# opendilab/DI-engine

Hardware: NVIDIA H100
Metric: learner transitions/sec (GAE+ppo_error fwd+bwd, T=128 x B=4096 per GPU) (higher is better)
Workload: dtype f32

## Files before the change

__graft_entry__.py:

```python
import os
import subprocess
import sys

ROOT = os.path.dirname(os.path.abspath(__file__))
if ROOT not in sys.path:
    sys.path.insert(0, ROOT)

CSRC = os.path.join(ROOT, 'di-engine_b200', 'csrc')
LIBDIR = os.path.join(ROOT, 'di-engine_b200', 'lib')
SOURCES = ['api.cu', 'gae.cu', 'ppo.cu', 'td.cu', 'pg.cu', 'fused.cu', 'colws.cu', 'vtws.cu', 'policy.cu', 'heads.cu',
           'quantile.cu', 'retrace.cu', 'acer.cu', 'vocab.cu', 'scatter.cu', 'lstm.cu']
ARCH = ['-gencode', 'arch=compute_90a,code=sm_90a']
NVCC_FLAGS = ARCH + [
    '-O3', '-lineinfo', '-std=c++17', '-Xcompiler', '-fPIC',
    '-Xcompiler', '-fvisibility=hidden', '--expt-extended-lambda'
]


def _stale(out, deps):
    if not os.path.isfile(out):
        return True
    t = os.path.getmtime(out)
    return any(os.path.getmtime(d) > t for d in deps)


def build(force=False):
    nvcc = os.environ.get('NVCC', 'nvcc')
    os.makedirs(LIBDIR, exist_ok=True)
    hdrs = [os.path.join(CSRC, h) for h in ('common.cuh', 'gae_tile.cuh', 'ppo_math.cuh', 'fused_args.cuh', 'policy_stats.cuh')]
    hdrs.append(os.path.join(ROOT, 'include', 'b200rl.h'))
    objs = []
    procs = []
    for src in SOURCES:
        s = os.path.join(CSRC, src)
        o = os.path.join(CSRC, src[:-3] + '.o')
        objs.append(o)
        if force or _stale(o, [s] + hdrs):
            procs.append((src, subprocess.Popen([nvcc] + NVCC_FLAGS + ['-c', s, '-o', o])))
    for src, p in procs:
        if p.wait() != 0:
            raise RuntimeError('nvcc failed on ' + src)
    out = os.path.join(LIBDIR, 'libb200rl.so')
    if force or procs or _stale(out, objs):
        subprocess.check_call([nvcc] + ARCH + ['-shared', '-o', out] + objs +
                              ['-lcudart'])
    build_c_example(force=force or bool(procs))
    from oracle import make_ref, ref_coma, ref_lm, ref_scatter
    make_ref.build()
    ref_lm.build()
    ref_coma.build()
    ref_scatter.build()
    import di_engine_b200
    lib = di_engine_b200._lib.load()
    assert lib.b200rl_built_for_sm() == 90
    return out


def build_c_example(force=False):
    src = os.path.join(ROOT, 'examples', 'c_abi_gae.c')
    exe = os.path.join(ROOT, 'examples', 'bin', 'c_abi_gae')
    lib = os.path.join(LIBDIR, 'libb200rl.so')
    if not force and not _stale(exe, [src, lib, os.path.join(ROOT, 'include', 'b200rl.h')]):
        return exe
    os.makedirs(os.path.dirname(exe), exist_ok=True)
    cuda = os.environ.get('CUDA_HOME', '/usr/local/cuda')
    subprocess.check_call([
        os.environ.get('CC', 'gcc'), '-std=c11', '-O2', '-ffp-contract=off', '-I', os.path.join(ROOT, 'include'), '-I',
        os.path.join(cuda, 'include'), src, '-L', LIBDIR, '-lb200rl', '-L', os.path.join(cuda, 'lib64'), '-lcudart',
        '-Wl,-rpath,$ORIGIN/../../di-engine_b200/lib', '-Wl,-rpath,' + os.path.join(cuda, 'lib64'), '-o', exe
    ])
    return exe


def smoke():
    import numpy as np
    import torch
    import di_engine_b200 as b2
    from oracle import rl_oracle
    from tests import cases
    assert torch.cuda.is_available(), 'smoke() needs a GPU'
    T, B, N = 128, 64, 6
    op, tg, pg = cases.gae_case(1, T, B, p_done=0.02)
# ... 32 lines not shown
```

di-engine_b200/csrc/policy.cu:

```cuda
#include <math.h>

#include "../../include/b200rl.h"
#include "policy_stats.cuh"

namespace b200rl {

constexpr int GS_NT = 1024;
constexpr int GS_MAX_T = 24576;

template <int VN>
__global__ void __launch_bounds__(GS_NT) gae_seq_kernel(const float* __restrict__ value, float* __restrict__ next_value,
                                                       const float* __restrict__ reward, const float* __restrict__ done,
                                                       const float* __restrict__ traj, float* __restrict__ adv, int T,
                                                       float gamma, float gl, int mask_inplace, RetArgs ra) {
    pdl_prologue();
    extern __shared__ float s_seq[];
    float* s_d = s_seq;
    float* s_f = s_seq + T;
    __shared__ int s_nseg;
    __shared__ int s_cnt[GS_NT / 32];
    const int tid = threadIdx.x;
    const float vs = ra.vscale;
    float mu = 0.f, sigma = 1.f;
    if constexpr (VN == VN_POPART) {
        mu = *ra.mu;
        sigma = *ra.sigma;
    }
    for (int t = tid; t < T; t += GS_NT) {
        const float v = vn_decode<VN>(value[t], vs);
        float nv = vn_decode<VN>(next_value[t], vs);
        float r = reward[t];
        if constexpr (VN == VN_POPART) r = __fdiv_rn(fsub(r, mu), sigma);
        const float d = done ? done[t] : 0.f;
        const float tf = traj ? traj[t] : d;
        if (done) {
            nv = fmul(nv, fsub(1.f, d));
            if (VN == VN_PPO && mask_inplace && d != 0.f) next_value[t] = nv;
        }
        s_d[t] = fsub(fadd(r, fmul(gamma, nv)), v);
        s_f[t] = fmul(gl, fsub(1.f, tf));
    }
    __syncthreads();
    const int strip = (T + GS_NT - 1) / GS_NT;
    const int t0 = tid * strip, t1 = min(T, t0 + strip);
    int mine = 0;
    for (int t = t0; t < t1; ++t) mine += (s_f[t] == 0.f || t == T - 1) ? 1 : 0;
    int incl = mine;
    const int lane = tid & 31, wid = tid >> 5;
#pragma unroll
    for (int o = 1; o < 32; o <<= 1) {
        const int n = __shfl_up_sync(0xffffffffu, incl, o);
        if (lane >= o) incl += n;
    }
    if (lane == 31) s_cnt[wid] = incl;
    __syncthreads();
// ... 92 lines not shown
    pdl_prologue();
    const float vs = ra.vscale;
    double acc[4] = {0.0, 0.0, 0.0, 0.0}, pv[2];
    const long long stride = (long long)gridDim.x * 256;
    long long i = (long long)blockIdx.x * 256 + threadIdx.x;
    if (VEC) {
        const long long n4 = n >> 2;
        const float4* v4 = reinterpret_cast<const float4*>(value);
        const float4* a4 = reinterpret_cast<const float4*>(adv);
        float4 v = make_float4(0.f, 0.f, 0.f, 0.f), a = v;
        if (i < n4) {
            v = v4[i];
            a = a4[i];
        }
        ret_pivots<VN>(vs, ret_value<VN>(ld_after_wait(value), vs), ld_after_wait(adv), pv);
        for (; i < n4; i += stride) {
            float4 ru, vo, ro;
            ret_one<VN>(vs, v.x, a.x, ru.x, vo.x, ro.x, acc, pv);
            ret_one<VN>(vs, v.y, a.y, ru.y, vo.y, ro.y, acc, pv);
            ret_one<VN>(vs, v.z, a.z, ru.z, vo.z, ro.z, acc, pv);
            ret_one<VN>(vs, v.w, a.w, ru.w, vo.w, ro.w, acc, pv);
            if (ra.ret_unnorm) reinterpret_cast<float4*>(ra.ret_unnorm)[i] = ru;
            if (ra.value_out) reinterpret_cast<float4*>(ra.value_out)[i] = vo;
            if (ra.ret_out) reinterpret_cast<float4*>(ra.ret_out)[i] = ro;
            if (i + stride < n4) {
                v = v4[i + stride];
                a = a4[i + stride];
            }
        }
    } else {
        float v = 0.f, a = 0.f;
        if (i < n) {
            v = value[i];
            a = adv[i];
        }
        ret_pivots<VN>(vs, ret_value<VN>(ld_after_wait(value), vs), ld_after_wait(adv), pv);
        for (; i < n; i += stride) {
            float ru, vo, ro;
            ret_one<VN>(vs, v, a, ru, vo, ro, acc, pv);
            if (ra.ret_unnorm) ra.ret_unnorm[i] = ru;
            if (ra.value_out) ra.value_out[i] = vo;
            if (ra.ret_out) ra.ret_out[i] = ro;
            if (i + stride < n) {
                v = value[i + stride];
                a = adv[i + stride];
            }
        }
    }
    if (!ra.stats && !ra.adv_stats) return;
    double tot[4];
    if (stats_grid_join<4, 256>(acc, tot, ws_part, ws_join)) write_ret_stats<VN>(ra, tot, pv, (double)n);
}

__global__ void __launch_bounds__(256) adv_stats_kernel(const float* __restrict__ x, long long n, float* __restrict__ out,
                                                        double* __restrict__ ws_part, unsigned int* __restrict__ ws_join) {
    pdl_prologue();
    const double p = stats_pivot(ld_after_wait(x));
    double acc[2] = {0.0, 0.0};
    for (long long i = (long long)blockIdx.x * 256 + threadIdx.x; i < n; i += (long long)gridDim.x * 256)
        moments_add(acc[0], acc[1], x[i], p);
    double tot[2];
    if (stats_grid_join<2, 256>(acc, tot, ws_part, ws_join)) write_adv_stats(out, tot[0], tot[1], p, (double)n);
}

__global__ void __launch_bounds__(256) normalize_kernel(const float* __restrict__ x, const float* __restrict__ stats,
                                                        long long n, float* __restrict__ out) {
    pdl_prologue();
    const float m = ld_after_wait(stats), d = ld_after_wait(stats + 1);
    for (long long i = (long long)blockIdx.x * 256 + threadIdx.x; i < n; i += (long long)gridDim.x * 256)
        out[i] = __fdiv_rn(fsub(x[i], m), d);
}

__global__ void __launch_bounds__(256) impala_mask_kernel(const float* __restrict__ values, const float* __restrict__ rewards,
                                                          const float* __restrict__ done, long long T, long long B,
                                                          float* __restrict__ values_out, float* __restrict__ rewards_out,
                                                          float* __restrict__ weights_out) {
    pdl_prologue();
    const long long n = (T + 1) * B;
    for (long long i = (long long)blockIdx.x * 256 + threadIdx.x; i < n; i += (long long)gridDim.x * 256) {
        const long long t = i / B;
        const float m = t >= 1 ? fsub(1.f, done[i - B]) : 1.f;
        values_out[i] = t >= 1 ? fmul(values[i], m) : values[i];
        if (t < T) {
            if (weights_out) weights_out[i] = m;
            if (rewards_out) rewards_out[i] = fmul(rewards[i], m);
        }
    }
}

enum ValueMap : int { VM_SYMLOG = 0, VM_INV_SYMLOG = 1, VM_H_INV = 2, VM_POPART_REWARD = 3 };

template <int M>
__device__ __forceinline__ float value_map(float x, float mu, float sigma) {
    if constexpr (M == VM_SYMLOG) return vn_symlog(x);
    else if constexpr (M == VM_INV_SYMLOG) return vn_inv_symlog(x);
    else if constexpr (M == VM_H_INV) return vn_h_inv(x);
    else return __fdiv_rn(fsub(x, mu), sigma);
}

template <int M>
__global__ void __launch_bounds__(256) value_map_kernel(const float* __restrict__ x0, float* __restrict__ y0,
                                                        const float* __restrict__ x1, float* __restrict__ y1, long long n,
                                                        const float* __restrict__ mu, const float* __restrict__ sigma) {
    pdl_prologue();
    float m = 0.f, sg = 1.f;
    if constexpr (M == VM_POPART_REWARD) {
        m = *mu;
        sg = *sigma;
    }
    for (long long i = (long long)blockIdx.x * 256 + threadIdx.x; i < n; i += (long long)gridDim.x * 256) {
        y0[i] = value_map<M>(x0[i], m, sg);
        if (x1) y1[i] = value_map<M>(x1[i], m, sg);
    }
}

template <int M>
__global__ void __launch_bounds__(256) value_map_bwd_kernel(const float* __restrict__ x, const float* __restrict__ g,
                                                            float* __restrict__ dx, long long n) {
    pdl_prologue();
    for (long long i = (long long)blockIdx.x * 256 + threadIdx.x; i < n; i += (long long)gridDim.x * 256) {
        const float xi = x[i], s = vn_sign(xi), gs = fmul(g[i], s);
        const float d = M == VM_SYMLOG ? __fdiv_rn(gs, fadd(fabsf(xi), 1.f)) : fmul(gs, expf(fabsf(xi)));
        dx[i] = fadd(0.f, fmul(d, s));
    }
}

}

using namespace b200rl;

namespace b200rl {
int gae_scan(const float* value, float* next_value, const float* reward, const float* done, const float* traj_flag, float* adv,
             long long T, long long C, long long A, double gamma_d, double lambda_d, int mask_next_value_inplace,
             float vscale, void* stream);
}

static double* ws_stats_part(float* ws) { return reinterpret_cast<double*>(ws + WS_CTRL_WORDS); }
static unsigned int* ws_joins(float* ws) { return reinterpret_cast<unsigned int*>(ws + WS_FX_OFF_WORDS + 48); }
static_assert(WS_CTRL_WORDS % 2 == 0 && WS_CTRL_WORDS + NUM_SMS * 8 * 4 * 2 <= WS_PARTIAL_LIMIT_WORDS,
              "the statistics rows fit the workspace's partial region");

extern "C" int b200rl_adv_stats(const float* x, long long n, float* stats2, float* workspace, size_t workspace_bytes,
                                void* stream) {
    if (!x || !stats2 || !workspace || n < 1 || workspace_bytes < WS_MIN_BYTES) return B200RL_ERR_ARG;
    long long grid = div_up(n, 256 * 8);
    if (grid > NUM_SMS * 4) grid = NUM_SMS * 4;
    if (grid < 1) grid = 1;
    return launch_k(adv_stats_kernel, (int)grid, 256, 0, (cudaStream_t)stream, x, n, stats2, ws_stats_part(workspace),
                    ws_joins(workspace));
}

extern "C" int b200rl_normalize(const float* x, const float* stats2, long long n, float* out, void* stream) {
    if (!x || !stats2 || !out || n < 0) return B200RL_ERR_ARG;
    if (n == 0) return B200RL_OK;
    long long grid = div_up(n, 256 * 4);
    if (grid > NUM_SMS * 8) grid = NUM_SMS * 8;
    return launch_k(normalize_kernel, (int)grid, 256, 0, (cudaStream_t)stream, x, stats2, n, out);
}

extern "C" int b200rl_gae_returns(const float* value, float* next_value, const float* reward, const float* done,
                                  const float* traj_flag, long long T, long long C, long long A, double gamma,
                                  double lambda_, int mask_next_value_inplace, double value_scale, float* adv,
                                  float* unnormalized_return, float* value_out, float* return_out, float* stats3,
                                  float* adv_stats2, float* workspace, size_t workspace_bytes, void* stream) {
    if (T < 1 || C < 1 || A < 1 || !value || !next_value || !reward || !adv || !workspace ||
        workspace_bytes < WS_MIN_BYTES || value_scale < 0.0)
        return B200RL_ERR_ARG;
    RetArgs ra{};
    ra.vscale = (float)value_scale;
    ra.ret_unnorm = unnormalized_return; ra.value_out = value_out; ra.ret_out = return_out; ra.stats = stats3;
    ra.adv_stats = adv_stats2;
    cudaStream_t st = (cudaStream_t)stream;
    if (C == 1 && T <= GS_MAX_T) {
        const size_t smem = (size_t)2 * T * sizeof(float);
        if (int rc = smem_opt_in<gae_seq_kernel<VN_PPO>>(smem)) return rc;
        return launch_k(gae_seq_kernel<VN_PPO>, 1, GS_NT, smem, st, value, next_value, reward, done, traj_flag, adv, (int)T,
                        (float)gamma, (float)(gamma * lambda_), mask_next_value_inplace, ra);
    }
    const bool want_epi = unnormalized_return || value_out || return_out || stats3 || adv_stats2;
    int rc = gae_scan(value, next_value, reward, done, traj_flag, adv, T, C, A, gamma, lambda_, mask_next_value_inplace,
                      (float)value_scale, stream);
    if (rc != 0 || !want_epi) return rc;
    const long long n = T * C;
    const bool vec = (n % 4 == 0) && aligned16(value) && aligned16(adv) && (!unnormalized_return || aligned16(unnormalized_return)) &&
                     (!value_out || aligned16(value_out)) && (!return_out || aligned16(return_out));
    long long grid = div_up(n, 256 * (vec ? 8 : 4));
    if (grid > NUM_SMS * 8) grid = NUM_SMS * 8;
    if (vec)
        return launch_k(returns_kernel<VN_PPO, true>, (int)grid, 256, 0, st, value, (const float*)adv, n, ra,
                        ws_stats_part(workspace), ws_joins(workspace));
    return launch_k(returns_kernel<VN_PPO, false>, (int)grid, 256, 0, st, value, (const float*)adv, n, ra,
                    ws_stats_part(workspace), ws_joins(workspace));
}

static long long map_grid(long long n) {
    long long grid = div_up(n, 256 * 4);
    if (grid > NUM_SMS * 8) grid = NUM_SMS * 8;
    return grid < 1 ? 1 : grid;
}

template <int VN>
static int launch_gae_seq(const float* value, const float* next_value, const float* reward, const float* done,
                          const float* traj_flag, float* adv, long long T, double gamma, double lambda_, const RetArgs& ra,
                          cudaStream_t st) {
    const size_t smem = (size_t)2 * T * sizeof(float);
    if (int rc = smem_opt_in<gae_seq_kernel<VN>>(smem)) return rc;
    return launch_k(gae_seq_kernel<VN>, 1, GS_NT, smem, st, value, const_cast<float*>(next_value), reward, done, traj_flag,
                    adv, (int)T, (float)gamma, (float)(gamma * lambda_), 0, ra);
}

template <int VN>
static int launch_returns(const float* value, const float* adv, long long n, const RetArgs& ra, float* workspace,
                          cudaStream_t st) {
    const bool vec = (n % 4 == 0) && aligned16(value) && aligned16(adv) && (!ra.value_out || aligned16(ra.value_out)) &&
                     (!ra.ret_out || aligned16(ra.ret_out));
    long long grid = div_up(n, 256 * (vec ? 8 : 4));
    if (grid > NUM_SMS * 8) grid = NUM_SMS * 8;
    if (vec)
        return launch_k(returns_kernel<VN, true>, (int)grid, 256, 0, st, value, adv, n, ra, ws_stats_part(workspace),
                        ws_joins(workspace));
    return launch_k(returns_kernel<VN, false>, (int)grid, 256, 0, st, value, adv, n, ra, ws_stats_part(workspace),
                    ws_joins(workspace));
}

template <int VN>
static int launch_gae_returns_tc(const float* value, const float* next_value, const float* reward, const float* done,
                                 const float* traj_flag, float* adv, long long T, long long C, double gamma, double lambda_,
                                 const RetArgs& ra, float* scratch, float* workspace, cudaStream_t st) {
    const long long n = T * C;
    const float* v = value;
    const float* nv = next_value;
    const float* r = reward;
    int rc = 0;
    if constexpr (VN == VN_RESCALE || VN == VN_SYMLOG) {
        constexpr int M = VN == VN_RESCALE ? VM_H_INV : VM_INV_SYMLOG;
        rc = launch_k(value_map_kernel<M>, (int)map_grid(n), 256, 0, st, value, scratch, next_value, scratch + n, n,
                      (const float*)nullptr, (const float*)nullptr);
        v = scratch;
        nv = scratch + n;
    } else if constexpr (VN == VN_POPART) {
        rc = launch_k(value_map_kernel<VM_POPART_REWARD>, (int)map_grid(n), 256, 0, st, reward, scratch,
                      (const float*)nullptr, (float*)nullptr, n, ra.mu, ra.sigma);
        r = scratch;
    }
    if (rc) return rc;
// ... 81 lines not shown
```

di-engine_b200/csrc/ppo.cu:

```cuda
#include "../../include/b200rl.h"
#include "ppo_math.cuh"

namespace b200rl {

constexpr int PS_CW = 8;
constexpr int PS_R = PS_CW * 32;
constexpr int PS_THREADS = PS_R + 32;
constexpr int PS_MAX_STAGES = 8;
constexpr int PS_AHEAD = 2;
constexpr size_t PS_SMEM_LIMIT = 227 * 1024 - 1024;
constexpr int PS_TRACE_STAGES = 56;

template <int NC, int WHAT>
__global__ void __launch_bounds__(PS_THREADS, 1) ppo_tile_kernel(PpoArgs a, float* ws, int n_stages, int trace) {
    extern __shared__ __align__(128) unsigned char smem[];
    unsigned long long* tr = trace ? reinterpret_cast<unsigned long long*>(ws + 65536) + blockIdx.x * 64 : nullptr;
    if (tr && threadIdx.x == 0) tr[0] = gtimer();
    pdl_prologue();
    if (tr && threadIdx.x == 0) tr[1] = gtimer();
    constexpr bool GRADS = (WHAT != PPO_FWD);
    constexpr bool LOSSES = (WHAT != PPO_BWD);
    const int N = NC ? NC : a.N;
    const int tid = threadIdx.x;
    const int wid = tid >> 5, lane = tid & 31;
    const bool has_pre = a.logit_pre != nullptr, has_w = a.weight != nullptr;
    const PpoTileLayout L = ppo_layout(N, has_pre, has_w, PS_R);
    const int NS = n_stages;
    uint64_t* full = reinterpret_cast<uint64_t*>(smem + NS * L.stage_bytes);
    uint64_t* empty = full + PS_MAX_STAGES;

    float g[4] = {0.f, 0.f, 0.f, 0.f};
    if (GRADS && upstream<4>(a.rec, WHAT == PPO_BWD, ppo_owned(a), g)) return;
    const PpoUpstream up{g[0], g[1], g[2], g[3], 1.f / (float)a.S};

    const long long n_full = a.S / PS_R;
    const int tail_rows = (int)(a.S - n_full * PS_R);
    const long long n_tiles = n_full + (tail_rows ? 1 : 0);
    const long long t0 = n_tiles * blockIdx.x / gridDim.x, t1 = n_tiles * (blockIdx.x + 1) / gridDim.x;
    const int my_n = (int)(t1 - t0);

    if (tid == 0) {
        for (int s = 0; s < NS; ++s) {
            mbar_init(&full[s], 1);
            mbar_init(&empty[s], PS_CW);
        }
        mbar_fence_init();
    }
    __syncthreads();

    float acc[6] = {0.f, 0.f, 0.f, 0.f, 0.f, 0.f};
    if (wid == PS_CW) {
        if (lane == 0) {
            for (int i = 0; i < my_n; ++i) {
                const long long t = t0 + i;
                if (t >= n_full) break;
                const int sg = i % NS;
                if (i >= NS) mbar_wait(&empty[sg], (uint32_t)(((i / NS) - 1) & 1));
                if (NS > PS_AHEAD && i >= PS_AHEAD) {
                    const int jb = i - PS_AHEAD;
                    mbar_wait(&full[jb % NS], (uint32_t)((jb / NS) & 1));
                }
                const long long row0 = t * PS_R;
                unsigned char* st = smem + sg * L.stage_bytes;
                uint64_t* bar = &full[sg];
                mbar_expect_tx(bar, (uint32_t)L.tx_bytes);
                tma_load_1d(st, a.logit_new + row0 * N, L.logit_bytes, bar);
                tma_load_1d(st + L.off_old, a.logit_old + row0 * N, L.logit_bytes, bar);
                if (has_pre) tma_load_1d(st + L.off_pre, a.logit_pre + row0 * N, L.logit_bytes, bar);
                tma_load_1d(st + L.off_act, a.action + row0, PS_R * 8, bar);
                tma_load_1d(st + L.off_vn, a.value_new + row0, PS_R * 4, bar);
                tma_load_1d(st + L.off_vo, a.value_old + row0, PS_R * 4, bar);
                tma_load_1d(st + L.off_adv, a.adv + row0, PS_R * 4, bar);
                tma_load_1d(st + L.off_ret, a.ret + row0, PS_R * 4, bar);
                if (has_w) tma_load_1d(st + L.off_w, a.weight + row0, PS_R * 4, bar);
            }
        }
    } else {
        const int rit = wid * 32 + lane;
        const int warp_out_bytes = 32 * N * 4;
        for (int i = 0; i < my_n; ++i) {
            const long long t = t0 + i;
            const long long row0 = t * PS_R;
            const int sg = i % NS;
            unsigned char* st = smem + sg * L.stage_bytes;
            const bool full_tile = t < n_full;
            if (full_tile) {
                mbar_wait(&full[sg], (uint32_t)((i / NS) & 1));
                if (tr && tid == 0) {
                    const unsigned long long now = gtimer();
                    if (i == 0) tr[2] = now;
                    tr[3] = now;
                    if (i < PS_TRACE_STAGES) tr[8 + i] = now;
                }
            } else if (rit < tail_rows) {
                float* d0 = reinterpret_cast<float*>(st) + rit * N;
                float* d1 = reinterpret_cast<float*>(st + L.off_old) + rit * N;
                float* d2 = reinterpret_cast<float*>(st + L.off_pre) + rit * N;
                for (int k = 0; k < N; ++k) {
                    d0[k] = a.logit_new[(row0 + rit) * N + k];
                    d1[k] = a.logit_old[(row0 + rit) * N + k];
                    if (has_pre) d2[k] = a.logit_pre[(row0 + rit) * N + k];
                }
                reinterpret_cast<long long*>(st + L.off_act)[rit] = a.action[row0 + rit];
                reinterpret_cast<float*>(st + L.off_vn)[rit] = a.value_new[row0 + rit];
                reinterpret_cast<float*>(st + L.off_vo)[rit] = a.value_old[row0 + rit];
                reinterpret_cast<float*>(st + L.off_adv)[rit] = a.adv[row0 + rit];
                reinterpret_cast<float*>(st + L.off_ret)[rit] = a.ret[row0 + rit];
                if (has_w) reinterpret_cast<float*>(st + L.off_w)[rit] = a.weight[row0 + rit];
            }
            if (full_tile || rit < tail_rows) {
                const float adv = reinterpret_cast<const float*>(st + L.off_adv)[rit];
                ppo_row_compute<NC, LOSSES, GRADS>(a, L, st, rit, N, adv, full_tile, reinterpret_cast<float*>(st), row0,
                                                   up, acc);
            }
            if (!full_tile) continue;
            if (GRADS) {
                fence_proxy_async_smem();
                __syncwarp();
                if (lane == 0) {
                    tma_store_1d(a.grad_logit + (row0 + wid * 32) * N, st + wid * warp_out_bytes, warp_out_bytes);
                    tma_store_commit();
                    if (NS == 1) {
                        tma_store_wait_read<0>();
                        mbar_arrive(&empty[sg]);
                    } else {
                        tma_store_wait_read<1>();
                        if (i > 0) mbar_arrive(&empty[(i - 1) % NS]);
// ... 155 lines not shown
    return a.G == 1 && a.N <= 32 && al;
}

template <int NT>
__global__ void __launch_bounds__(NT) ppo_value_kernel(const float* __restrict__ value_new,
                                                       const float* __restrict__ value_old,
                                                       const float* __restrict__ ret, const float* __restrict__ weight,
                                                       long long S, float clip, int use_clip, float* __restrict__ out,
                                                       float* __restrict__ dvalue, float* ws) {
    pdl_prologue();
    float acc[1] = {0.f};
    const float inv_s = 1.f / (float)S;
    for (long long i = (long long)blockIdx.x * NT + threadIdx.x; i < S; i += (long long)gridDim.x * NT) {
        const float w = weight ? weight[i] : 1.f;
        float d;
        const float t = value_term(value_new[i], use_clip ? value_old[i] : 0.f, ret[i], clip, use_clip, d);
        acc[0] += t * w;
        if (dvalue) dvalue[i] = 0.5f * w * inv_s * d;
    }
    double tot[1];
    if (grid_sum<1, NT>(acc, tot, ws, 0) && threadIdx.x == 0) out[0] = (float)(0.5 * tot[0] / (double)S);
}

struct PsGeo {
    int grid, stages;
    size_t smem;
};
static PsGeo ps_pick(long long S, int N, bool has_pre, bool has_w, bool verify_only, int sm_count) {
    PsGeo g{};
    const size_t stage = (size_t)ppo_layout(N, has_pre, has_w, PS_R).stage_bytes;
    const size_t bars = 2 * PS_MAX_STAGES * sizeof(uint64_t);
    const long long n_tiles = (S + PS_R - 1) / PS_R;
    g.grid = (int)(n_tiles < sm_count ? n_tiles : sm_count);
    const long long per_cta = g.grid > 0 ? (n_tiles + g.grid - 1) / g.grid : 0;
    long long stages = verify_only ? 1 : (long long)((PS_SMEM_LIMIT - bars) / stage);
    if (stages > PS_MAX_STAGES) stages = PS_MAX_STAGES;
    if (stages > per_cta) stages = per_cta;
    g.stages = stages < 1 ? 0 : (int)stages;
    g.smem = (size_t)g.stages * stage + bars;
    return g;
}

template <int NC, int WHAT>
static int launch_tile(const PpoArgs& a, float* out, float* ws, size_t ws_bytes, cudaStream_t st) {
    int sm_count = 0;
    if (int rc = sm_count_of(sm_count)) return rc;
    const PsGeo g = ps_pick(a.S, a.N, a.logit_pre != nullptr, a.weight != nullptr, WHAT == PPO_BWD && a.rec.used, sm_count);
    if (g.stages < 1) return B200RL_ERR_ARG;
    constexpr auto kern = ppo_tile_kernel<NC, WHAT>;
    if (int rc = smem_opt_in<kern>(g.smem)) return rc;
    if (WHAT != PPO_BWD && !ws_partials_fit((long long)g.grid * 6, ws_bytes)) return B200RL_ERR_WORKSPACE;
    const int trace = WHAT != PPO_BWD && trace_enabled();
    if (trace && (size_t)65536 * 4 + (size_t)g.grid * 64 * 8 > ws_bytes) return B200RL_ERR_WORKSPACE;
    if (int rc = launch_k(kern, g.grid, PS_THREADS, g.smem, st, a, ws, g.stages, trace)) return rc;
    if (WHAT == PPO_BWD) return B200RL_OK;
    return launch_finalize(ws, out, ppo_finalize_args(a.S, a.logit_pre != nullptr, g.grid), st);
}

template <int WHAT>
static int dispatch_tile(const PpoArgs& a, float* out, float* ws, size_t ws_bytes, cudaStream_t st) {
    return with_nc(a.N, [&](auto nc) { return launch_tile<nc, WHAT>(a, out, ws, ws_bytes, st); });
}

}

using namespace b200rl;

static int fill_args(PpoArgs& a, const float* logit_new, const float* logit_old, const float* logit_pretrained,
                     const long long* action, const float* value_new, const float* value_old, const float* adv,
                     const float* return_, const float* weight, long long S, long long G, long long N,
                     double clip_ratio, int use_value_clip, double dual_clip, int kl_type, const float* adv_stats,
                     const float* factor) {
    a.adv_stats = adv_stats;
    a.factor = factor;
    a.logit_new = logit_new; a.logit_old = logit_old; a.logit_pre = logit_pretrained; a.action = action;
    a.value_new = value_new; a.value_old = value_old; a.adv = adv; a.ret = return_; a.weight = weight;
    a.S = S; a.G = (int)G; a.N = (int)N; a.clip = (float)clip_ratio; a.clip_lo = (float)(1.0 - clip_ratio);
    a.clip_hi = (float)(1.0 + clip_ratio); a.dual_clip = (float)dual_clip;
    a.use_value_clip = use_value_clip; a.kl_type = kl_type;
    if (S < 0 || G < 1 || N < 1) return B200RL_ERR_ARG;
    if (!logit_new || !logit_old || !action || !value_new || !value_old || !adv || !return_) return B200RL_ERR_ARG;
    if (kl_type < 1 || kl_type > 3) return B200RL_ERR_ARG;
    return B200RL_OK;
}

extern "C" int b200rl_ppo_fwd(const float* logit_new, const float* logit_old, const float* logit_pretrained,
                              const long long* action, const float* value_new, const float* value_old,
                              const float* adv, const float* return_, const float* weight, long long S, long long G,
                              long long N, double clip_ratio, int use_value_clip, double dual_clip, int kl_type,
                              const float* adv_stats, const float* factor, float* out, float* workspace,
                              size_t workspace_bytes, void* stream) {
    PpoArgs a{};
    int rc = fill_args(a, logit_new, logit_old, logit_pretrained, action, value_new, value_old, adv, return_, weight,
                       S, G, N, clip_ratio, use_value_clip, dual_clip, kl_type, adv_stats, factor);
    if (rc != B200RL_OK || !out || !workspace) return rc != B200RL_OK ? rc : B200RL_ERR_ARG;
    if (S == 0) return B200RL_ERR_ARG;
    cudaStream_t st = (cudaStream_t)stream;
    if (tile_path_ok(a)) return dispatch_tile<PPO_FWD>(a, out, workspace, workspace_bytes, st);
    constexpr int NT = 128;
    const bool warp = a.N > 64;
    int grid = warp ? div_up(S, NT / 32) : div_up(S, NT);
    if (grid > NUM_SMS * 16) grid = NUM_SMS * 16;
    if (!ws_partials_fit((long long)((size_t)grid * 6), workspace_bytes)) return B200RL_ERR_WORKSPACE;
    if (warp) return launch_k(ppo_fwd_kernel<NT, 2>, grid, NT, 0, st, a, out, workspace);
    return launch_k(ppo_fwd_kernel<NT, 1>, grid, NT, 0, st, a, out, workspace);
}

extern "C" int b200rl_ppo_fwd_grad(const float* logit_new, const float* logit_old, const float* logit_pretrained,
                                   const long long* action, const float* value_new, const float* value_old,
// ... 84 lines not shown
```

Before: 22.09 billion.

## Fuse GAE scan with returns epilogue in a warp-specialized column kernel; prefetch PPO inputs before PDL wait

Replaces the separate GAE scan and returns/stats kernels with one column-tiled kernel. Producer warps cp.async chunks backward in time, compute deltas and run the per-column scan in shared memory, while consumer warps compute returns and statistics and stream the outputs through an mbarrier ring. A side warp computes the first-row pivots for the stats. The PPO tile kernel now issues TMA loads for inputs the GAE kernel does not write before the grid-dependency wait, so those loads overlap the previous kernel when chain analysis allows it. This adds new synchronization, shared-memory budgeting for co-residency and chain-tracking logic.

```diff
diff --git a/__graft_entry__.py b/__graft_entry__.py
--- a/__graft_entry__.py
+++ b/__graft_entry__.py
@@ -27,7 +27,8 @@
 def build(force=False):
     nvcc = os.environ.get('NVCC', 'nvcc')
     os.makedirs(LIBDIR, exist_ok=True)
-    hdrs = [os.path.join(CSRC, h) for h in ('common.cuh', 'gae_tile.cuh', 'ppo_math.cuh', 'fused_args.cuh', 'policy_stats.cuh')]
+    hdrs = [os.path.join(CSRC, h) for h in ('common.cuh', 'gae_tile.cuh', 'gae_chunk.cuh', 'ppo_math.cuh', 'fused_args.cuh',
+                                          'policy_stats.cuh')]
     hdrs.append(os.path.join(ROOT, 'include', 'b200rl.h'))
     objs = []
     procs = []
diff --git a/di-engine_b200/csrc/gae_chunk.cuh b/di-engine_b200/csrc/gae_chunk.cuh
--- /dev/null
+++ b/di-engine_b200/csrc/gae_chunk.cuh
@@ -0,0 +1,140 @@
+#pragma once
+#include "common.cuh"
+
+namespace b200rl {
+
+struct GaeIn {
+    const float* value;
+    float* next_value;
+    const float* reward;
+    const float* done;
+    const float* traj;
+};
+
+__device__ __forceinline__ void cpa4(void* smem_dst, const void* gmem_src) {
+    asm volatile("cp.async.ca.shared.global [%0], [%1], 4;" ::"r"(smem_u32(smem_dst)), "l"(gmem_src) : "memory");
+}
+
+template <int TC, int R, bool VEC>
+__device__ __forceinline__ void gae_chunk_issue(unsigned char* dst, const GaeIn& g, long long C, long long A, long long t0,
+                                                long long c0, int W, int lane) {
+    constexpr int ARR = R * TC * 4;
+    if constexpr (VEC) {
+        constexpr int PR = TC / 4;
+        static_assert(R * PR % 32 == 0, "whole pieces per lane");
+#pragma unroll
+        for (int k = 0; k < R * PR / 32; ++k) {
+            const int p = lane + 32 * k;
+            const int row = p / PR, o = p % PR;
+            if (t0 + row >= 0 && o * 4 < W) {
+                const long long off = (t0 + row) * C + c0 + o * 4;
+                cpa16(dst + p * 16, g.value + off);
+                cpa16(dst + ARR + p * 16, g.next_value + off);
+                cpa16(dst + 2 * ARR + p * 16, g.reward + off);
+                if (g.done) cpa16(dst + 3 * ARR + p * 16, g.done + off);
+                if (g.traj) cpa16(dst + 4 * ARR + p * 16, g.traj + off);
+            }
+        }
+    } else {
+        static_assert(R * TC % 32 == 0, "whole elements per lane");
+        const long long Caux = C / A;
+#pragma unroll
+        for (int k = 0; k < R * TC / 32; ++k) {
+            const int e = lane + 32 * k;
+            const int row = e / TC, col = e % TC;
+            if (t0 + row >= 0 && col < W) {
+                const long long off = (t0 + row) * C + c0 + col;
+                const long long aoff = (t0 + row) * Caux + (c0 + col) / A;
+                cpa4(dst + e * 4, g.value + off);
+                cpa4(dst + ARR + e * 4, g.next_value + off);
+                cpa4(dst + 2 * ARR + e * 4, g.reward + aoff);
+                if (g.done) cpa4(dst + 3 * ARR + e * 4, g.done + aoff);
+                if (g.traj) cpa4(dst + 4 * ARR + e * 4, g.traj + aoff);
+            }
+        }
+    }
+}
+
+template <int TC, int R, bool VEC>
+__device__ __forceinline__ void gae_chunk_delta(const float* rv, float (*ab)[TC], float (*fb)[TC], float (*vk)[TC],
+                                                const GaeIn& g, float gamma, float gl, float vscale, int mask_inplace,
+                                                bool skip_col0, long long C, long long t0, long long c0, int lane) {
+    constexpr int PR = TC / 4;
+    const bool has_done = g.done != nullptr, has_traj = g.traj != nullptr;
+    const float* rn = rv + R * TC;
+    const float* rr = rn + R * TC;
+    const float* rd = rr + R * TC;
+    const float* rt = rd + R * TC;
+    const int cq = (lane % PR) * 4;
+#pragma unroll
+    for (int p = 0; p < R * PR / 32; ++p) {
+        const int jj = p * (32 / PR) + lane / PR;
+        const long long t = t0 + jj;
+        if (t >= 0 && c0 + cq < C) {
+            const int o = jj * TC + cq;
+            const float4 v4 = *reinterpret_cast<const float4*>(rv + o);
+            const float4 n4 = *reinterpret_cast<const float4*>(rn + o);
+            const float4 r4 = *reinterpret_cast<const float4*>(rr + o);
+            const float4 d4 = has_done ? *reinterpret_cast<const float4*>(rd + o) : make_float4(0.f, 0.f, 0.f, 0.f);
+            const float4 t4 = has_traj ? *reinterpret_cast<const float4*>(rt + o) : d4;
+            float vv[4] = {v4.x, v4.y, v4.z, v4.w}, nn[4] = {n4.x, n4.y, n4.z, n4.w};
+            float rw[4] = {r4.x, r4.y, r4.z, r4.w}, dd[4] = {d4.x, d4.y, d4.z, d4.w};
+            float tt[4] = {t4.x, t4.y, t4.z, t4.w};
+            if (vk) *reinterpret_cast<float4*>(&vk[jj][cq]) = v4;
+            float de[4], fa[4];
+            bool changed = false;
+#pragma unroll
+            for (int k = 0; k < 4; ++k) {
+                if (vscale != 0.f) {
+                    vv[k] = fmul(vv[k], vscale);
+                    nn[k] = fmul(nn[k], vscale);
+                }
+                if (has_done) {
+                    changed |= (dd[k] != 0.f);
+                    nn[k] = fmul(nn[k], fsub(1.f, dd[k]));
+                }
+                de[k] = fsub(fadd(rw[k], fmul(gamma, nn[k])), vv[k]);
+                fa[k] = fmul(gl, fsub(1.f, tt[k]));
+            }
+            *reinterpret_cast<float4*>(&ab[jj][cq]) = make_float4(de[0], de[1], de[2], de[3]);
+            *reinterpret_cast<float4*>(&fb[jj][cq]) = make_float4(fa[0], fa[1], fa[2], fa[3]);
+            if (changed && mask_inplace) {
+                float* dst = g.next_value + t * C + c0 + cq;
+                if (VEC && !(skip_col0 && c0 + cq == 0)) {
+                    *reinterpret_cast<float4*>(dst) = make_float4(nn[0], nn[1], nn[2], nn[3]);
+                } else {
+#pragma unroll
+                    for (int k = 0; k < 4; ++k)
+                        if (c0 + cq + k < C && !(skip_col0 && c0 + cq + k == 0)) dst[k] = nn[k];
+                }
+            }
+        }
+    }
+}
+
+template <int TC, int R>
+__device__ __forceinline__ void gae_chunk_scan(float (*ab)[TC], const float (*fb)[TC], float& carry, long long C, long long t0,
+                                               long long c0, int lane) {
+    if (lane < TC && c0 + lane < C) {
+        if (t0 >= 0) {
+            float d[R], g[R];
+#pragma unroll
+            for (int k = 0; k < R; ++k) {
+                d[k] = ab[R - 1 - k][lane];
+                g[k] = fb[R - 1 - k][lane];
+            }
+#pragma unroll
+            for (int k = 0; k < R; ++k) {
+                carry = fadd(d[k], fmul(g[k], carry));
+                ab[R - 1 - k][lane] = carry;
+            }
+        } else {
+            for (int jj = R - 1; jj >= 0 && t0 + jj >= 0; --jj) {
+                carry = fadd(ab[jj][lane], fmul(fb[jj][lane], carry));
+                ab[jj][lane] = carry;
+            }
+        }
+    }
+}
+
+}
diff --git a/di-engine_b200/csrc/policy.cu b/di-engine_b200/csrc/policy.cu
--- a/di-engine_b200/csrc/policy.cu
+++ b/di-engine_b200/csrc/policy.cu
@@ -1,6 +1,7 @@
 #include <math.h>
 
 #include "../../include/b200rl.h"
+#include "gae_chunk.cuh"
 #include "policy_stats.cuh"
 
 namespace b200rl {
@@ -199,6 +200,221 @@
     if (stats_grid_join<4, 256>(acc, tot, ws_part, ws_join)) write_ret_stats<VN>(ra, tot, pv, (double)n);
 }
 
+constexpr int GR_TC = 32;
+constexpr int GR_EW = 8;
+constexpr int GR_R = GR_EW * 32 / GR_TC;
+constexpr int GR_THREADS = GR_EW * 32 + 64;
+constexpr int GR_RAWS = 8;
+constexpr int GR_S = 8;
+constexpr int GR_PTC = 4, GR_PR = 32;
+constexpr int GR_PRAWS = 4;
+constexpr int GR_ARR = GR_R * GR_TC * 4;
+constexpr int GR_PARR = GR_PR * GR_PTC * 4;
+constexpr size_t GR_SMEM = (size_t)GR_RAWS * 5 * GR_ARR + 2 * GR_S * GR_ARR + GR_ARR + (size_t)GR_PRAWS * 5 * GR_PARR +
+                           2 * GR_PARR + (2 * GR_S + 1) * sizeof(uint64_t);
+constexpr size_t GR_STATIC_SMEM = 512;
+static_assert(GR_SMEM + GR_STATIC_SMEM + (8 * 256 * (2 * 6 * 4 + 8 + 4 * 4) + 2 * 8 * 8 + 256) + 2 * 1024 <= 228 * 1024,
+              "gae_returns_col_kernel and the PPO launch behind it share an SM");
+constexpr int GR_TRACE_WORD = 98304;
+constexpr int GR_TRACE_CHUNKS = 56;
+
+struct GrItem {
+    long long tile;
+    long long q;
+};
+
+template <bool VEC>
+__global__ void __launch_bounds__(GR_THREADS, 1)
+    gae_returns_col_kernel(GaeIn g, float* __restrict__ adv, long long T, long long C, long long A, float gamma, float gl,
+                           int mask_inplace, int defer_wait, RetArgs ra, double* __restrict__ ws_part,
+                           unsigned int* __restrict__ ws_join, unsigned long long* __restrict__ trace) {
+    extern __shared__ __align__(128) unsigned char smem[];
+    unsigned char* raw = smem;
+    auto advs = reinterpret_cast<float (*)[GR_R][GR_TC]>(raw + GR_RAWS * 5 * GR_ARR);
+    auto vals = advs + GR_S;
+    auto fbuf = reinterpret_cast<float (*)[GR_TC]>(vals + GR_S);
+    unsigned char* praw = reinterpret_cast<unsigned char*>(fbuf + GR_R);
+    auto pab = reinterpret_cast<float (*)[GR_PTC]>(praw + GR_PRAWS * 5 * GR_PARR);
+    auto pfb = pab + GR_PR;
+    uint64_t* ready = reinterpret_cast<uint64_t*>(pfb + GR_PR);
+    uint64_t* freed = ready + GR_S;
+    uint64_t* pv_ready = freed + GR_S;
+    __shared__ double s_pv[2];
+    __shared__ int s_fin;
+    const int tid = threadIdx.x, wid = tid >> 5, lane = tid & 31;
+    const float vs = ra.vscale;
+    const bool stats = ra.stats || ra.adv_stats;
+    const bool skip0 = stats && mask_inplace;
+    const long long n_tiles = (C + GR_TC - 1) / GR_TC, n_chunks = (T + GR_R - 1) / GR_R;
+    const long long tile0 = n_tiles * blockIdx.x / gridDim.x, tile1 = n_tiles * (blockIdx.x + 1) / gridDim.x;
+    unsigned long long* tr = trace ? trace + blockIdx.x * 64 : nullptr;
+    if (tid == 0) {
+        if (tr) tr[0] = gtimer();
+        for (int s = 0; s < GR_S; ++s) {
+            mbar_init(&ready[s], 1);
+            mbar_init(&freed[s], GR_EW);
+        }
+        mbar_init(pv_ready, 1);
+        mbar_fence_init();
+    }
+    __syncthreads();
+    auto dep_wait = [] {
+        asm volatile("griddepcontrol.wait;" ::: "memory");
+        asm volatile("griddepcontrol.launch_dependents;" ::: "memory");
+    };
+    if (!defer_wait) dep_wait();
+    auto item_valid = [&](const GrItem& it) { return it.tile < tile1; };
+    auto item_next = [&](GrItem& it) {
+        if (++it.q >= n_chunks) {
+            it.q = 0;
+            ++it.tile;
+        }
+    };
+    const GrItem first{tile0, 0};
+    auto tile_w = [&](long long c0) { return (int)(C - c0 < GR_TC ? C - c0 : GR_TC); };
+    double acc[4] = {0.0, 0.0, 0.0, 0.0}, pv[2] = {0.0, 0.0};
+
+    if (wid == GR_EW) {
+        auto issue = [&](const GrItem& it, int slot) {
+            const long long c0 = it.tile * GR_TC;
+            gae_chunk_issue<GR_TC, GR_R, VEC>(raw + slot * 5 * GR_ARR, g, C, A, T - (it.q + 1) * GR_R, c0, tile_w(c0), lane);
+        };
+        GrItem it = first, pf = first;
+        for (int k = 0; k < GR_RAWS; ++k) {
+            if (item_valid(pf)) {
+                issue(pf, k);
+                item_next(pf);
+            }
+            cpa_commit();
+        }
+        if (defer_wait) dep_wait();
+        float carry = 0.f;
+        int s = 0, ph = 0;
+        for (int j = 0; item_valid(it); ++j) {
+            const long long c0 = it.tile * GR_TC;
+            const long long t0 = T - (it.q + 1) * GR_R;
+            const int slot = j % GR_RAWS;
+            if (it.q == 0) carry = 0.f;
+            cpa_wait<GR_RAWS - 1>();
+            __syncwarp();
+            if (tr && lane == 0 && j == 0) tr[2] = gtimer();
+            if (j >= GR_S) mbar_wait(&freed[s], (uint32_t)(ph ^ 1));
+            gae_chunk_delta<GR_TC, GR_R, VEC>(reinterpret_cast<const float*>(raw + slot * 5 * GR_ARR), advs[s], fbuf, vals[s],
+                                              g, gamma, gl, vs, mask_inplace, skip0, C, t0, c0, lane);
+            __syncwarp();
+            if (item_valid(pf)) {
+                issue(pf, slot);
+                item_next(pf);
+            }
+            cpa_commit();
+            gae_chunk_scan<GR_TC, GR_R>(advs[s], fbuf, carry, C, t0, c0, lane);
+            __syncwarp();
+            if (lane == 0) {
+                mbar_arrive(&ready[s]);
+                if (tr) {
+                    const unsigned long long now = gtimer();
+                    tr[3] = now;
+                    if (j < GR_TRACE_CHUNKS) tr[8 + j] = now;
+                }
+            }
+            if (++s == GR_S) { s = 0; ph ^= 1; }
+            item_next(it);
+        }
+        cpa_wait<0>();
+    } else if (wid == GR_EW + 1) {
+        if (stats) {
+            const long long pn = (T + GR_PR - 1) / GR_PR;
+            auto issue = [&](long long q, int slot) {
+                gae_chunk_issue<GR_PTC, GR_PR, VEC>(praw + slot * 5 * GR_PARR, g, C, A, T - (q + 1) * GR_PR, 0, 1, lane);
+            };
+            long long pq = 0;
+            for (int k = 0; k < GR_PRAWS; ++k) {
+                if (pq < pn) issue(pq++, k);
+                cpa_commit();
+            }
+            float carry = 0.f;
+            for (long long q = 0; q < pn; ++q) {
+                const int slot = (int)(q % GR_PRAWS);
+                const long long t0 = T - (q + 1) * GR_PR;
+                cpa_wait<GR_PRAWS - 1>();
+                __syncwarp();
+                gae_chunk_delta<GR_PTC, GR_PR, VEC>(reinterpret_cast<const float*>(praw + slot * 5 * GR_PARR), pab, pfb,
+                                                    nullptr, g, gamma, gl, vs, 0, false, C, t0, 0, lane);
+                __syncwarp();
+                if (pq < pn) issue(pq++, slot);
+                cpa_commit();
+                gae_chunk_scan<GR_PTC, GR_PR>(pab, pfb, carry, C, t0, 0, lane);
+                __syncwarp();
+            }
+            cpa_wait<0>();
+            unsigned long long ready_at = 0;
+            if (lane == 0) {
+                double p[2];
+                ret_pivots<VN_PPO>(vs, ret_value<VN_PPO>(__ldcg(g.value), vs), carry, p);
+                s_pv[0] = p[0];
+                s_pv[1] = p[1];
+                mbar_arrive(pv_ready);
+                if (tr) ready_at = gtimer();
+            }
+            if (defer_wait) dep_wait();
+            if (tr && lane == 0) tr[6] = ready_at;
+        } else if (defer_wait) {
+            dep_wait();
+        }
+    } else {
+        if (defer_wait) dep_wait();
+        if (tr && tid == 0) tr[1] = gtimer();
+        if (stats) {
+            mbar_wait(pv_ready, 0);
+            pv[0] = s_pv[0];
+            pv[1] = s_pv[1];
+        }
+        const int jj = tid / GR_TC, c = tid % GR_TC;
+        GrItem it = first;
+        int s = 0, ph = 0;
+        while (item_valid(it)) {
+            const long long c0 = it.tile * GR_TC;
+            const long long t = T - (it.q + 1) * GR_R + jj;
+            mbar_wait(&ready[s], (uint32_t)ph);
+            if (t >= 0 && c0 + c < C) {
+                const float a = advs[s][jj][c];
+                const long long i = t * C + c0 + c;
+                float ru, vo, ro;
+                ret_one<VN_PPO>(vs, vals[s][jj][c], a, ru, vo, ro, acc, pv);
+                stg_stream(adv + i, a);
+                if (ra.ret_unnorm) stg_stream(ra.ret_unnorm + i, ru);
+                if (ra.value_out) stg_stream(ra.value_out + i, vo);
+                if (ra.ret_out) stg_stream(ra.ret_out + i, ro);
+            }
+            __syncwarp();
+            if (lane == 0) mbar_arrive(&freed[s]);
+            if (++s == GR_S) { s = 0; ph ^= 1; }
+            item_next(it);
+        }
+        if (tr && tid == 0) {
+            tr[4] = gtimer();
+            tr[5] = (unsigned long long)smid() << 32 | (unsigned long long)((tile1 - tile0) * n_chunks);
+        }
+    }
+    if (!stats) return;
+    double tot[4];
+    const bool fin = stats_grid_join<4, GR_THREADS>(acc, tot, ws_part, ws_join);
+    if (fin) write_ret_stats<VN_PPO>(ra, tot, pv, (double)T * (double)C);
+    if (!skip0 || !g.done) return;
+    if (tid == 0) s_fin = fin;
+    __syncthreads();
+    if (!s_fin) return;
+    const long long Caux = C / A;
+    for (long long t = tid; t < T; t += GR_THREADS) {
+        const float d = g.done[t * Caux];
+        if (d != 0.f) {
+            float nv = g.next_value[t * C];
+            if (vs != 0.f) nv = fmul(nv, vs);
+            g.next_value[t * C] = fmul(nv, fsub(1.f, d));
+        }
+    }
+}
+
 __global__ void __launch_bounds__(256) adv_stats_kernel(const float* __restrict__ x, long long n, float* __restrict__ out,
                                                         double* __restrict__ ws_part, unsigned int* __restrict__ ws_join) {
     pdl_prologue();
@@ -303,6 +519,49 @@
     long long grid = div_up(n, 256 * 4);
     if (grid > NUM_SMS * 8) grid = NUM_SMS * 8;
     return launch_k(normalize_kernel, (int)grid, 256, 0, (cudaStream_t)stream, x, stats2, n, out);
+}
+
+static int launch_gae_returns_col(const float* value, float* next_value, const float* reward, const float* done,
+                                  const float* traj, float* adv, long long T, long long C, long long A, double gamma,
+                                  double lambda_, int mask_inplace, const RetArgs& ra, float* ws, size_t ws_bytes,
+                                  cudaStream_t st) {
+    if (C % A != 0) return B200RL_ERR_ARG;
+    int sm_count = 0;
+    if (int rc = sm_count_of(sm_count)) return rc;
+    const long long n_tiles = (C + GR_TC - 1) / GR_TC;
+    long long grid = n_tiles < sm_count ? n_tiles : sm_count;
+    if (grid > NUM_SMS * 8) grid = NUM_SMS * 8;
+    const bool vec = A == 1 && C % 4 == 0 && aligned16(value) && aligned16(next_value) && aligned16(reward) &&
+                     (!done || aligned16(done)) && (!traj || aligned16(traj));
+    const long long F = T * C * 4, Fa = T * (C / A) * 4;
+    const ByteSpan reads[] = {byte_span(value, F), byte_span(next_value, F), byte_span(reward, Fa), byte_span(done, Fa),
+                              byte_span(traj, Fa)};
+    const ChainPoint at = capture_now(st);
+    const int defer = chain_may_defer(st, at, reads, 5) ? 1 : 0;
+    unsigned long long* trace = nullptr;
+    if (trace_enabled()) {
+        if ((size_t)(GR_TRACE_WORD + grid * 128) * 4 > ws_bytes) return B200RL_ERR_WORKSPACE;
+        trace = reinterpret_cast<unsigned long long*>(ws + GR_TRACE_WORD);
+    }
+    const GaeIn g{value, next_value, reward, done, traj};
+    const float gm = (float)gamma, gl = (float)(gamma * lambda_);
+    int rc;
+    if (vec) {
+        if ((rc = smem_opt_in<gae_returns_col_kernel<true>>(GR_SMEM))) return rc;
+        rc = launch_k(gae_returns_col_kernel<true>, (int)grid, GR_THREADS, GR_SMEM, st, g, adv, T, C, A, gm, gl, mask_inplace,
+                      defer, ra, ws_stats_part(ws), ws_joins(ws), trace);
+    } else {
+        if ((rc = smem_opt_in<gae_returns_col_kernel<false>>(GR_SMEM))) return rc;
+        rc = launch_k(gae_returns_col_kernel<false>, (int)grid, GR_THREADS, GR_SMEM, st, g, adv, T, C, A, gm, gl,
+                      mask_inplace, defer, ra, ws_stats_part(ws), ws_joins(ws), trace);
+    }
+    if (rc) return rc;
+    const ByteSpan writes[] = {byte_span(adv, F),          byte_span(ra.ret_unnorm, F),
+                               byte_span(ra.value_out, F), byte_span(ra.ret_out, F),
+                               byte_span(ra.stats, 12),    byte_span(ra.adv_stats, 8),
+                               byte_span(ws, (long long)ws_bytes), byte_span(mask_inplace ? next_value : nullptr, F)};
+    chain_report(st, at, true, writes, 8);
+    return B200RL_OK;
 }
 
 extern "C" int b200rl_gae_returns(const float* value, float* next_value, const float* reward, const float* done,
@@ -324,20 +583,8 @@
         return launch_k(gae_seq_kernel<VN_PPO>, 1, GS_NT, smem, st, value, next_value, reward, done, traj_flag, adv, (int)T,
                         (float)gamma, (float)(gamma * lambda_), mask_next_value_inplace, ra);
     }
-    const bool want_epi = unnormalized_return || value_out || return_out || stats3 || adv_stats2;
-    int rc = gae_scan(value, next_value, reward, done, traj_flag, adv, T, C, A, gamma, lambda_, mask_next_value_inplace,
-                      (float)value_scale, stream);
-    if (rc != 0 || !want_epi) return rc;
-    const long long n = T * C;
-    const bool vec = (n % 4 == 0) && aligned16(value) && aligned16(adv) && (!unnormalized_return || aligned16(unnormalized_return)) &&
-                     (!value_out || aligned16(value_out)) && (!return_out || aligned16(return_out));
-    long long grid = div_up(n, 256 * (vec ? 8 : 4));
-    if (grid > NUM_SMS * 8) grid = NUM_SMS * 8;
-    if (vec)
-        return launch_k(returns_kernel<VN_PPO, true>, (int)grid, 256, 0, st, value, (const float*)adv, n, ra,
-                        ws_stats_part(workspace), ws_joins(workspace));
-    return launch_k(returns_kernel<VN_PPO, false>, (int)grid, 256, 0, st, value, (const float*)adv, n, ra,
-                    ws_stats_part(workspace), ws_joins(workspace));
+    return launch_gae_returns_col(value, next_value, reward, done, traj_flag, adv, T, C, A, gamma, lambda_,
+                                  mask_next_value_inplace, ra, workspace, workspace_bytes, st);
 }
 
 static long long map_grid(long long n) {
diff --git a/di-engine_b200/csrc/ppo.cu b/di-engine_b200/csrc/ppo.cu
--- a/di-engine_b200/csrc/ppo.cu
+++ b/di-engine_b200/csrc/ppo.cu
@@ -12,12 +12,10 @@
 constexpr int PS_TRACE_STAGES = 56;
 
 template <int NC, int WHAT>
-__global__ void __launch_bounds__(PS_THREADS, 1) ppo_tile_kernel(PpoArgs a, float* ws, int n_stages, int trace) {
+__global__ void __launch_bounds__(PS_THREADS, 1) ppo_tile_kernel(PpoArgs a, float* ws, int n_stages, int trace, int early) {
     extern __shared__ __align__(128) unsigned char smem[];
     unsigned long long* tr = trace ? reinterpret_cast<unsigned long long*>(ws + 65536) + blockIdx.x * 64 : nullptr;
     if (tr && threadIdx.x == 0) tr[0] = gtimer();
-    pdl_prologue();
-    if (tr && threadIdx.x == 0) tr[1] = gtimer();
     constexpr bool GRADS = (WHAT != PPO_FWD);
     constexpr bool LOSSES = (WHAT != PPO_BWD);
     const int N = NC ? NC : a.N;
@@ -29,10 +27,6 @@
     uint64_t* full = reinterpret_cast<uint64_t*>(smem + NS * L.stage_bytes);
     uint64_t* empty = full + PS_MAX_STAGES;
 
-    float g[4] = {0.f, 0.f, 0.f, 0.f};
-    if (GRADS && upstream<4>(a.rec, WHAT == PPO_BWD, ppo_owned(a), g)) return;
-    const PpoUpstream up{g[0], g[1], g[2], g[3], 1.f / (float)a.S};
-
     const long long n_full = a.S / PS_R;
     const int tail_rows = (int)(a.S - n_full * PS_R);
     const long long n_tiles = n_full + (tail_rows ? 1 : 0);
@@ -47,6 +41,33 @@
         mbar_fence_init();
     }
     __syncthreads();
+    auto issue_static = [&](unsigned char* st, long long row0, uint64_t* bar) {
+        tma_load_1d(st, a.logit_new + row0 * N, L.logit_bytes, bar);
+        tma_load_1d(st + L.off_old, a.logit_old + row0 * N, L.logit_bytes, bar);
+        if (has_pre) tma_load_1d(st + L.off_pre, a.logit_pre + row0 * N, L.logit_bytes, bar);
+        tma_load_1d(st + L.off_act, a.action + row0, PS_R * 8, bar);
+        tma_load_1d(st + L.off_vn, a.value_new + row0, PS_R * 4, bar);
+        if (has_w) tma_load_1d(st + L.off_w, a.weight + row0, PS_R * 4, bar);
+    };
+    auto issue_written = [&](unsigned char* st, long long row0, uint64_t* bar) {
+        tma_load_1d(st + L.off_vo, a.value_old + row0, PS_R * 4, bar);
+        tma_load_1d(st + L.off_adv, a.adv + row0, PS_R * 4, bar);
+        tma_load_1d(st + L.off_ret, a.ret + row0, PS_R * 4, bar);
+    };
+    int n_early = 0;
+    if (early && wid == PS_CW && lane == 0) {
+        for (; n_early < PS_AHEAD && n_early < NS && n_early < my_n && t0 + n_early < n_full; ++n_early) {
+            uint64_t* bar = &full[n_early];
+            mbar_expect_tx(bar, (uint32_t)L.tx_bytes);
+            issue_static(smem + n_early * L.stage_bytes, (t0 + n_early) * PS_R, bar);
+        }
+    }
+    pdl_prologue();
+    if (tr && threadIdx.x == 0) tr[1] = gtimer();
+
+    float g[4] = {0.f, 0.f, 0.f, 0.f};
+    if (GRADS && upstream<4>(a.rec, WHAT == PPO_BWD, ppo_owned(a), g)) return;
+    const PpoUpstream up{g[0], g[1], g[2], g[3], 1.f / (float)a.S};
 
     float acc[6] = {0.f, 0.f, 0.f, 0.f, 0.f, 0.f};
     if (wid == PS_CW) {
@@ -63,16 +84,11 @@
                 const long long row0 = t * PS_R;
                 unsigned char* st = smem + sg * L.stage_bytes;
                 uint64_t* bar = &full[sg];
-                mbar_expect_tx(bar, (uint32_t)L.tx_bytes);
-                tma_load_1d(st, a.logit_new + row0 * N, L.logit_bytes, bar);
-                tma_load_1d(st + L.off_old, a.logit_old + row0 * N, L.logit_bytes, bar);
-                if (has_pre) tma_load_1d(st + L.off_pre, a.logit_pre + row0 * N, L.logit_bytes, bar);
-                tma_load_1d(st + L.off_act, a.action + row0, PS_R * 8, bar);
-                tma_load_1d(st + L.off_vn, a.value_new + row0, PS_R * 4, bar);
-                tma_load_1d(st + L.off_vo, a.value_old + row0, PS_R * 4, bar);
-                tma_load_1d(st + L.off_adv, a.adv + row0, PS_R * 4, bar);
-                tma_load_1d(st + L.off_ret, a.ret + row0, PS_R * 4, bar);
-                if (has_w) tma_load_1d(st + L.off_w, a.weight + row0, PS_R * 4, bar);
+                if (i >= n_early) {
+                    mbar_expect_tx(bar, (uint32_t)L.tx_bytes);
+                    issue_static(st, row0, bar);
+                }
+                issue_written(st, row0, bar);
             }
         }
     } else {
@@ -334,9 +350,24 @@
     if (WHAT != PPO_BWD && !ws_partials_fit((long long)g.grid * 6, ws_bytes)) return B200RL_ERR_WORKSPACE;
     const int trace = WHAT != PPO_BWD && trace_enabled();
     if (trace && (size_t)65536 * 4 + (size_t)g.grid * 64 * 8 > ws_bytes) return B200RL_ERR_WORKSPACE;
-    if (int rc = launch_k(kern, g.grid, PS_THREADS, g.smem, st, a, ws, g.stages, trace)) return rc;
+    const ChainPoint at = WHAT == PPO_FWD_GRAD ? capture_now(st) : ChainPoint{};
+    int early = 0;
+    if (WHAT == PPO_FWD_GRAD) {
+        const long long S = a.S, Lb = S * a.N * 4;
+        const ByteSpan reads[] = {byte_span(a.logit_new, Lb), byte_span(a.logit_old, Lb), byte_span(a.logit_pre, Lb),
+                                  byte_span(a.action, S * 8), byte_span(a.value_new, S * 4), byte_span(a.weight, S * 4)};
+        early = chain_may_defer(st, at, reads, 6) ? 1 : 0;
+    }
+    if (int rc = launch_k(kern, g.grid, PS_THREADS, g.smem, st, a, ws, g.stages, trace, early)) return rc;
     if (WHAT == PPO_BWD) return B200RL_OK;
-    return launch_finalize(ws, out, ppo_finalize_args(a.S, a.logit_pre != nullptr, g.grid), st);
+    if (int rc = launch_finalize(ws, out, ppo_finalize_args(a.S, a.logit_pre != nullptr, g.grid), st)) return rc;
+    if (WHAT == PPO_FWD_GRAD) {
+        const ByteSpan w[] = {byte_span(a.grad_logit, a.S * a.N * 4), byte_span(a.grad_value, a.S * 4),
+                              byte_span(a.rec.used, 4 * sizeof(float)), byte_span(out, 8 * sizeof(float)),
+                              byte_span(ws, (long long)ws_bytes)};
+        chain_report(st, at, false, w, 5);
+    }
+    return B200RL_OK;
 }
 
 template <int WHAT>
```

After: 22.07 billion, median of 6. About the same (-0.1%).
